# ryanelandt/PressureFieldContact.jl

Hardware: AMD Instinct MI355X
Metric: tet-tri clip+integrate ops/s (higher is better)
Workload: dtype f64

## Files before the change

### pressurefieldcontact.jl_amd/csrc/pfc_hip.hip

```cpp
#include "pfc_kernels.h"

#include <atomic>
#include <condition_variable>
#include <functional>
#include <mutex>
#include <thread>
#include <cmath>
#include <cstdlib>
#include <limits>
#include <cstdarg>
#include <cstdio>
#include <cstring>
#include <string>
#include <vector>

#include "../../include/pfc.h"
#include "pfc_sort.h"

namespace pfc {

__global__ void k_prep_tri(int n, const double *__restrict__ pt, const int *__restrict__ tri, TriRec *__restrict__ out) {
    int k = blockIdx.x * blockDim.x + threadIdx.x;
    if (k >= n) return;
    V3 a = ld3(pt + 3 * tri[3 * k]), b = ld3(pt + 3 * tri[3 * k + 1]), c = ld3(pt + 3 * tri[3 * k + 2]);
// ... 329 lines not shown
    hipStream_t last_stream = nullptr;
    long long stats[8] = {0, 0, 0, 0, 0, 0, 0, 0};
    DevBuf<double> dual_in, dual_acc, dual_res, dual_out, dual_poly;
    DevBuf<int2> dual_pkey;
    DevBuf<int> dual_sel, dual_flag;
    DevBuf<double> scat_d;
    DevBuf<int> scat_i;
    DevBuf<double> sdual_d, sdual_w;
    DevBuf<int> sdual_i;
    DevBuf<char> sdual_tmp;
    DevBuf<int> surv;
    DevBuf<int> rgn;
    DevBuf<int> poly_item, pcnt, poly_cand;
    DevBuf<double> poly;
    long long last_undecided = 0;
    long long last_active = 0;
    struct ShapeHint { int n = 0; bool sparse = false; } hints[4];
    void note_shape(int n, bool sparse) {
        int k = 0;
        while (k < 3 && hints[k].n != n) ++k;
        for (; k > 0; --k) hints[k] = hints[k - 1];
        hints[0].n = n; hints[0].sparse = sparse;
    }
    bool shape_is_sparse(int n) const {
        for (const ShapeHint &e : hints) if (e.n == n) return e.sparse;
        return false;
    }
    long long last_tslots = 0;
    Event ev[EV_COUNT];
    bool ev_valid = false;
    pfc_context *twin = nullptr;
    bool is_twin = false;
    DevBuf<int> fout;
    PinBuf<int> h_fout;
    int *fout_dev = nullptr;
    const int *fout_host = nullptr;
    int opt_fused = 1;
    int opt_fixed_order = 0;
    DevBuf<int> det;
    DevBuf<unsigned long long> sort_keys[2];
    DevBuf<int> canon_off, canon_fill, canon_item;
    int sort_tmp_items = 0;
    bool fixed_whole_list = false;
    DevBuf<char> sort_tmp;
    size_t sort_tmp_for = 0;
    int sort_tmp_bits = 0;
    int max_elem1 = 1, max_elem2 = 1;
    DevBuf<double> fx_rec, vfx_rec;
    DevBuf<int> vfx_head;
    DevBuf<int> fx_head;
    long long surv_sorted_serial = -1;
    size_t sort_cover = 0;
    size_t sort_cover_used = 0;
    int opt_clip_queue = 1;
    int fused_skip = 0;
    int fused_seq = 0;
    int fu_nw = 1;
    int last_fu_nw = 0, last_team = 0;
    int n_cu = 0;
    int opt_team = 48;
    DevBuf<unsigned long long> team;
    DevBuf<int> emit_ctr;
    PinBuf<int> h_emit;
    PinBuf<unsigned> h_more;
    bool fu_emit = false;
    int dual_fused_skip = 0;
    const double *fu_dpose = nullptr, *fu_dtwist = nullptr;
    double *fu_dwrench = nullptr, *fu_dsdot = nullptr;
    int fu_ndir = 0;
    bool pending_fused = false, last_fused = false;
    int opt_split_min = 1025;
    int opt_clip_min = 384;
    int opt_poison = 0;
    int split_n0 = 0;
    bool in_split = false;
    int last_parts = 1;
    Event ev_fork, ev_join, ev_join0;
    int twin_queue_fallback = 0;
    DevBuf<long long> surf_cnt, surf_off, surf_out;
    DevBuf<double> surf_part;
    DevBuf<int> surf_seg, surf_canon_off, surf_canon_fill, surf_canon_item;
    DevBuf<double> ljac_seed;
    DevBuf<double> ljac_out;
    DevBuf<double> ljac_io;
    DevBuf<int> ljac_ids;
    DevBuf<unsigned long long> surf_keys[2];
    DevBuf<char> surf_tmp;
    PinBuf<long long> h_surf;
    bool pending_surface = false;
    bool surf_whole_list = false;
    bool surf_cap_short = false;
    int surf_n_ctr = 0;
    long long surf_cap_poly = 0, surf_cap_trac = 0;
    DevBuf<long long> surf_hl;
    DevBuf<int> surf_hi;
    DevBuf<double> surf_hd, surf_in;
    size_t surf_hcap_poly = 0, surf_hcap_trac = 0;
    DevBuf<double> sfric_mom, sfric_sum, sfric_res;
    DevBuf<double> sfric_hd;
};

namespace {

int fail(pfc_context *h, int code, const char *fmt, ...) {
    char buf[512];
    va_list ap;
// ... 278 lines not shown
    } else if (np_mode == 0) {
        if (h->any_tet_tet) hipLaunchKernelGGL((k_narrow<true, 0>), dim3(np_grid), dim3(kNpBlock), 0, st, np);
        else hipLaunchKernelGGL((k_narrow<false, 0>), dim3(np_grid), dim3(kNpBlock), 0, st, np);
    } else {
        if (h->opt_clip_queue && !h->any_tet_tet) {
            hipLaunchKernelGGL(k_clip_queue, dim3(np_grid), dim3(kNpBlock), 0, st, np);
        } else if (h->in_split || (n_items >= 640 && n_items < 1024)) {
            if (h->any_tet_tet) hipLaunchKernelGGL((k_narrow<true, 3>), dim3(np_grid), dim3(kNpBlock), 0, st, np);
            else hipLaunchKernelGGL((k_narrow<false, 3>), dim3(np_grid), dim3(kNpBlock), 0, st, np);
        } else {
            if (h->any_tet_tet) hipLaunchKernelGGL((k_narrow<true, 2>), dim3(np_grid), dim3(kNpBlock), 0, st, np);
            else hipLaunchKernelGGL((k_narrow<false, 2>), dim3(np_grid), dim3(kNpBlock), 0, st, np);
        }
        IntegArgs ig;
        ig.items = h->items.p; ig.n_items = n_items; ig.ccount = ccount; ig.ccap = (int)h->ccap; ig.chunk_switch = kNpChunkSwitch;
        ig.pcnt = h->pcnt.p; ig.poly_item = h->poly_item.p; ig.poly = h->poly.p; ig.pcap = np.pcap;
        ig.poly_cand = np.poly_cand; ig.surv = np.surv; ig.scount = np.scount; ig.acc = h->acc.p; ig.rec = h->rec.p;
        ig.rgn = h->rgn.p; ig.rr_cap = np.rr_cap; ig.icnt = h->icnt.p; ig.status = h->status.p;
        ig.det = h->opt_fixed_order ? h->det.p : nullptr;
        if (h->opt_fixed_order) hipLaunchKernelGGL(k_integ_fixed, dim3(grid_for(h->ccap, 64, kNpMaxBlocks)), dim3(64), 0, st, ig);
        else hipLaunchKernelGGL(k_integ, dim3(grid_for(h->ccap, 64, kNpMaxBlocks)), dim3(64), 0, st, ig);
    }
    if (prof) HIP_TRY(h, hipEventRecord(h->ev[EV_NP], st));

    BrArgs br;
    br.items = h->items.p; br.n_items = n_items; br.acc = h->acc.p; br.res = h->res.p; br.icnt = h->icnt.p;
    br.trac = trac_view(h); br.tcount = tcount; br.tcap = (int)h->tcap; br.wrench = d_wrench; br.sdot = d_sdot;
    br.counts = d_counts;
    br.ctr = h->ctr.p; br.n_ctr = levels + 12; br.status = h->status.p; br.tail = h->tail_dev ? h->tail_dev : h->tail.p;
    br.rgn = h->rgn.p; br.i_pcount = (levels + 9) & ~1;
    if (h->opt_fixed_order && np_mode == 2) {
        FixedArgs fx;
        fx.rec = h->rec.p; fx.det = h->det.p; fx.n_items = n_items; fx.n_slots = (int)(h->rcap / kRgn) * kRgn; fx.items = h->items.p;
        fx.acc = h->acc.p; fx.status = h->status.p;
        hipLaunchKernelGGL(k_shift_fixed, dim3(n_items), dim3(64), 0, st, fx);
    }
    if (h->any_bristle) {
        ShiftArgs sh;
        sh.rec = h->rec.p; sh.rgn = h->rgn.p; sh.rr_cap = (int)(h->rcap / kRgn); sh.acc = h->acc.p;
        if (!(h->opt_fixed_order && np_mode == 2)) hipLaunchKernelGGL(k_shift, dim3(grid_for(h->rcap, 64, 2048)), dim3(64), 0, st, sh);
        hipLaunchKernelGGL(k_eig, dim3(n_items), dim3(64), 0, st, br);
        FricArgs fr;
        fr.items = h->items.p; fr.poly_item = h->poly_item.p; fr.poly = h->poly.p; fr.ccount = ccount; fr.ccap = (int)h->ccap;
        fr.chunk_switch = kNpChunkSwitch; fr.pcnt = h->pcnt.p;
        fr.pcap = np.pcap; fr.res = h->res.p; fr.acc = h->acc.p;
        fr.n_items = n_items; fr.status = h->status.p;
        fr.sink = FixedSink{nullptr, nullptr, nullptr, 0, 0, 0, 0, 0, nullptr};
        if (h->opt_fixed_order && np_mode == 2) {
            const size_t n_pos = h->ccap / 64 + 1, cap = fixed_fric_cap(h->ccap, n_items);
            HIP_TRY(h, hipMemsetAsync(h->vfx_head.p, 0xFF, sizeof(int) * (size_t)n_items, st));
            HIP_TRY(h, hipMemsetAsync(h->vfx_head.p + n_items, 0, sizeof(int) * 2, st));
            fr.sink = FixedSink{h->vfx_rec.p, h->vfx_head.p + n_items, h->vfx_head.p, 0, 2, (int)n_pos, (int)(2 * n_pos), (int)cap, h->status.p};
        }
        if (fr.sink.rec) {
            hipLaunchKernelGGL(k_fric_fixed, dim3(grid_for(h->ccap, 64, 256 * 32)), dim3(64), 0, st, fr);
            hipLaunchKernelGGL(k_fixed_reduce, dim3(n_items), dim3(64), 0, st, fr.sink, n_items, h->acc.p, kAccStride, kAccFric, 6);
        } else hipLaunchKernelGGL(k_fric, dim3(grid_for(h->ccap, 64, 256 * 32)), dim3(64), 0, st, fr);
    }
    if (prof) HIP_TRY(h, hipEventRecord(h->ev[EV_BR], st));
    hipLaunchKernelGGL(k_final, dim3(grid_for(n_items, 128, 1 << 20)), dim3(128), 0, st, br);
    if (prof) HIP_TRY(h, hipEventRecord(h->ev[EV_FIN], st));
    HIP_TRY(h, hipGetLastError());
    return PFC_OK;
}

int enqueue_eval(pfc_context *h, int n_items, const int *d_ins_ids, const double *d_pose, const double *d_twist,
                 const double *d_s, double *d_wrench, double *d_sdot, int *d_counts, hipStream_t st) {
    new_value_pass(h);
    h->pending_more = false; h->last_dual_reused = false;
    HIP_TRY(h, ensure_work(h, n_items));
    const int levels = eff_levels(h);
    const bool prof = h->opt_profile != 0;
    if (prof && !h->ev[0])
        for (int k = 0; k < EV_COUNT; ++k) HIP_TRY(h, hipEventCreate(h->ev[k].put()));
    const int L = bfs_levels_for(h, n_items, levels);
    bool use_graph = h->opt_graph && !prof;
#ifdef PFC_STAMPS
    use_graph = false;
#endif
    if (use_graph) {
        pfc_context::GraphKey key = {};
        key.n_items = n_items; key.levels = levels; key.L = L; key.debug = (h->opt_debug ? 1 : 0) | (h->in_split ? 2 : 0) | (bp_block_for(h, n_items) << 4);
        if (h->opt_fixed_order) {
            size_t cover = h->sort_cover ? h->sort_cover : h->ccap;
            int lg = 0;
            while (((size_t)1 << lg) < cover && lg < 40) ++lg;
            key.debug |= ((lg + 1) << 16) | (h->fixed_whole_list ? 1 << 24 : 0);
        }
        key.bristle = (h->any_bristle ? 1 : 0) | (h->any_tet_tet ? 2 : 0);
        key.surv = h->want_surv ? 1 : 0;
        key.p[0] = d_ins_ids; key.p[1] = d_pose; key.p[2] = d_twist; key.p[3] = d_s; key.p[4] = d_wrench;
        key.p[5] = d_sdot; key.p[6] = d_counts; key.p[7] = h->tail_dev; key.p[8] = h->bp_dev; key.stream = (void *)st; key.epoch = h->epoch;
        const int gi = key.surv;
        if (!h->ghave[gi] || std::memcmp(&key, &h->gkey[gi], sizeof key) != 0) {
            h->gexec[gi].reset();
            h->ghave[gi] = false;
            hipGraph_t graph = nullptr;
            HIP_TRY(h, hipStreamBeginCapture(st, hipStreamCaptureModeThreadLocal));
            int rc = record_eval(h, n_items, d_ins_ids, d_pose, d_twist, d_s, d_wrench, d_sdot, d_counts, st, false);
            hipError_t e = hipStreamEndCapture(st, &graph);
            if (rc != PFC_OK) { if (graph) (void)hipGraphDestroy(graph); return rc; }
            if (e != hipSuccess) return fail(h, PFC_ERR_HIP, "hipStreamEndCapture failed: %s", hipGetErrorString(e));
            e = hipGraphInstantiate(h->gexec[gi].put(), graph, nullptr, nullptr, 0);
            (void)hipGraphDestroy(graph);
            if (e != hipSuccess) return fail(h, PFC_ERR_HIP, "hipGraphInstantiate failed: %s", hipGetErrorString(e));
            h->gkey[gi] = key; h->ghave[gi] = true;
        }
        HIP_TRY(h, hipGraphLaunch(h->gexec[gi], st));
    } else {
        int rc = record_eval(h, n_items, d_ins_ids, d_pose, d_twist, d_s, d_wrench, d_sdot, d_counts, st, prof);
// ... 672 lines not shown
        HIP_TRY(h, copy_sync(h, h->d_insfull, full.data(), sizeof(InsFull) * full.size(), hipMemcpyHostToDevice));
    }
    h->finalized = true;
    return PFC_OK;
}

static int check_eval_args(pfc_context *h, int n_items, const void *ins_ids, const void *pose, const void *twist,
                           const void *s, const void *wrench, const void *sdot) {
    if (!h->finalized) return fail(h, PFC_ERR_STATE, "pfc_eval before pfc_finalize");
    if (n_items < 0) return fail(h, PFC_ERR_BAD_ARG, "negative n_items");
    if (n_items == 0) return PFC_OK;
    if (h->ins.empty()) return fail(h, PFC_ERR_STATE, "no contact instructions");
    if (!pose || !twist || !wrench || !sdot) return fail(h, PFC_ERR_BAD_ARG, "null buffer");
    if (!ins_ids && n_items > (int)h->ins.size())
        return fail(h, PFC_ERR_BAD_ARG, "n_items exceeds the number of instructions and no ins_ids given");
    if (h->any_bristle && !s) return fail(h, PFC_ERR_BAD_ARG, "bristle instructions need the state buffer s");
    return PFC_OK;
}

int pfc_eval_device(pfc_handle h, int n_items, const int *d_ins_ids, const double *d_pose, const double *d_twist,
                    const double *d_s, double *d_wrench, double *d_sdot, int *d_counts, void *stream) {
    if (!h) return PFC_ERR_BAD_ARG;
    if (h->multi)
        return multi_eval_device(h, n_items, 0, d_ins_ids, d_pose, nullptr, d_twist, d_s, nullptr, nullptr, nullptr, d_wrench, d_sdot,
                                 nullptr, nullptr, d_counts, stream);
    { const int rc = check_eval_args(h, n_items, d_ins_ids, d_pose, d_twist, d_s, d_wrench, d_sdot); if (rc != PFC_OK) return rc; }
    if (n_items == 0) { h->pending = false; h->last_n_items = 0; return PFC_OK; }
    HIP_TRY(h, hipSetDevice(h->device));
    hipStream_t st = stream ? (hipStream_t)stream : h->stream;
    h->split_n0 = 0;
    h->pending_fused = false;
    end_kept_pass(h);
    h->pending_more = false;
    int team = fused_team(h, n_items);
    if (team > 1 && !team_acquire(h)) team = fused_ok(h, n_items) ? 1 : 0;
    if (team) {
        h->fu_nw = team;
        const int rc_t = enqueue_fused(h, n_items, d_ins_ids, d_pose, d_twist, d_s, d_wrench, d_sdot, d_counts, st);
        h->fu_nw = 1;
        if (rc_t != PFC_OK) team_release(h);
        return rc_t;
    }
    if (h->fused_skip > 0 && n_items <= kFusedMaxItems) --h->fused_skip;
    const bool split = h->opt_split_min > 0 && n_items >= h->opt_split_min && d_ins_ids && !h->opt_debug && !h->opt_fixed_order &&
                       !h->want_surv && !h->is_twin && !pile_mode(h, n_items);
    if (!split) return enqueue_eval(h, n_items, d_ins_ids, d_pose, d_twist, d_s, d_wrench, d_sdot, d_counts, st);
    int rc = make_twin(h);
    if (rc != PFC_OK) return rc;
    pfc_context *t = h->twin;
    t->opt_profile = h->opt_profile; t->opt_max_levels = h->opt_max_levels; t->opt_bfs_levels = h->opt_bfs_levels;
    t->opt_poison = h->opt_poison;
    if (t->opt_clip_min != h->opt_clip_min) { t->opt_clip_min = h->opt_clip_min; t->ghave[0] = t->ghave[1] = false; }
    if (t->opt_clip_queue != h->opt_clip_queue) { t->opt_clip_queue = h->opt_clip_queue; t->ghave[0] = t->ghave[1] = false; }
    t->opt_graph = h->opt_graph;
    if (t->opt_no_filter != h->opt_no_filter) { t->opt_no_filter = h->opt_no_filter; t->ghave[0] = t->ghave[1] = false; }
    const int n0 = n_items / 2, n1 = n_items - n0;
    hipStream_t s0 = h->stream;
    HIP_TRY(h, hipEventRecord(h->ev_fork, st));
    if (s0 != st) HIP_TRY(h, hipStreamWaitEvent(s0, h->ev_fork, 0));
    HIP_TRY(h, hipStreamWaitEvent(t->stream, h->ev_fork, 0));
    h->in_split = true; t->in_split = true;
    rc = enqueue_eval(h, n0, d_ins_ids, d_pose, d_twist, d_s, d_wrench, d_sdot, d_counts, s0);
    h->in_split = false;
    if (rc != PFC_OK) return rc;
    rc = enqueue_eval(t, n1, d_ins_ids + n0, d_pose + 24 * (size_t)n0, d_twist + 6 * (size_t)n0,
                      d_s ? d_s + 6 * (size_t)n0 : nullptr, d_wrench + 6 * (size_t)n0, d_sdot + 6 * (size_t)n0,
                      d_counts ? d_counts + 4 * (size_t)n0 : nullptr, t->stream);
    if (rc != PFC_OK) { h->err = t->err; return rc; }
    HIP_TRY(h, hipEventRecord(h->ev_join, t->stream));
    HIP_TRY(h, hipStreamWaitEvent(st, h->ev_join, 0));
    if (s0 != st) {
        HIP_TRY(h, hipEventRecord(h->ev_join0, s0));
        HIP_TRY(h, hipStreamWaitEvent(st, h->ev_join0, 0));
    }
    h->split_n0 = n0;
    return PFC_OK;
}

namespace {

struct SurfFricOut {
    const double *s;
    double *fric, *fric_summary, *stiff;
};

int surface_enqueue(pfc_context *h, int n_items, const int *d_ins_ids, const double *d_pose, const double *d_twist, long long cap_poly,
                    long long cap_trac, long long *d_poly_off, int *d_poly_idx, double *d_poly_xyz, long long *d_poly_trac,
                    double *d_trac, double *d_summary, int *d_counts, long long *d_totals, hipStream_t st, const SurfFricOut *fo = nullptr) {
    new_value_pass(h);
    h->pending_more = false;
    h->pin_in_pt = {}; h->pin_din_pt = {};
    h->pending = false; h->pending_dual = false; h->pending_dual_hyb = false; h->split_n0 = 0;
    if (h->pending_fused) { h->pending_fused = false; team_release(h); }
    int ba, bb;
    const int bits = pfc_sort_key_bits(n_items, h->max_elem1, h->max_elem2, &ba, &bb);
    if (bits > 64)
        return fail(h, PFC_ERR_BAD_ARG, "pfc_contact_surface: (item, element, element) needs %d key bits for %d items, more than 64", bits, n_items);
    HIP_TRY(h, ensure_work(h, n_items));
    const size_t c = h->ccap;
    HIP_TRY(h, h->surf_cnt.ensure(2 * (c + 1)));
    HIP_TRY(h, h->surf_off.ensure(2 * (c + 1)));
    HIP_TRY(h, h->surf_part.ensure(c * kSurfSums));
    HIP_TRY(h, h->surf_seg.ensure((size_t)n_items + 1));
    HIP_TRY(h, h->surf_canon_off.ensure((size_t)n_items + 1));
    HIP_TRY(h, h->surf_canon_fill.ensure((size_t)n_items));
    HIP_TRY(h, h->surf_canon_item.ensure(c));
// ... 1172 lines not shown
        copy_out_dual(po + n * 12, nk, d_wrench, d_sdot);
        h->dual_counts_cache.assign(pc, pc + n * 4);
        h->pin_din_pt = {n_items, ins_ids != nullptr, h->value_serial, in_d};
        return PFC_OK;
    }
    h->want_surv = true;
    int rc = pfc_eval(h, n_items, ins_ids, pose, twist, s, wrench, sdot, counts);
    h->want_surv = false;
    if (rc != PFC_OK) return rc;
    HIP_TRY(h, ensure_graphed(h, h->dual_in, nk * 36));
    HIP_TRY(h, ensure_graphed(h, h->dual_acc, nk * kDaStride));
    HIP_TRY(h, ensure_graphed(h, h->dual_res, nk * kDrStride));
    HIP_TRY(h, ensure_graphed(h, h->dual_out, nk * 12));
    double *dp = h->dual_in.p, *dt = dp + nk * 24, *dsd = dt + nk * 6;
    const size_t in_bytes = sizeof(double) * nk * 36, out_bytes = sizeof(double) * nk * 12;
    HIP_TRY(h, h->pin_in.ensure(in_bytes));
    HIP_TRY(h, h->pin_out.ensure(out_bytes));
    pack_seeds((double *)h->pin_in.p, nk, d_pose, d_twist, d_s, true);
    HIP_TRY(h, hipMemcpyAsync(dp, h->pin_in.p, in_bytes, hipMemcpyHostToDevice, st));
    rc = launch_dual(h, n_items, n_dir, h->tail.p, dp, dt, dsd, h->dual_out.p, h->dual_out.p + nk * 6, (size_t)h->stats[2], st, nullptr);
    if (rc != PFC_OK) return rc;
    h->dual_hint = h->stats[2];
    HIP_TRY(h, hipMemcpyAsync(h->pin_out.p, h->dual_out.p, out_bytes, hipMemcpyDeviceToHost, st));
    HIP_TRY(h, hipStreamSynchronize(st));
    copy_out_dual((const double *)h->pin_out.p, nk, d_wrench, d_sdot);
    return PFC_OK;
}

int pfc_set_option(pfc_handle h, const char *name, long long value) {
    if (!h || !name) return PFC_ERR_BAD_ARG;
    if (h->multi) {
        if (!std::strcmp(name, "multi_min")) { h->multi->opt_min_items = value < 1 ? 1 : (int)value; h->multi->part_n = 0; return PFC_OK; }
        h->multi->dev_kept = false;
        for (pfc_context *c : h->multi->shard) {
            const int rc = on_shard(h, c, [&](pfc_context *c1) { return pfc_set_option(c1, name, value); });
            if (rc != PFC_OK) return rc;
        }
        return PFC_OK;
    }
    end_kept_pass(h);
    if (!std::strcmp(name, "debug")) h->opt_debug = value != 0;
    else if (!std::strcmp(name, "profile")) h->opt_profile = value != 0;
    else if (!std::strcmp(name, "max_levels")) {
        if (value < 0 || value > (1 << 20) || (h->finalized && value > h->max_levels))
            return fail(h, PFC_ERR_BAD_ARG, "max_levels must be 0 (automatic) or 1..%d (depth of the finalized trees + 1)", h->max_levels);
        h->opt_max_levels = (int)value; h->ghave[0] = h->ghave[1] = false; h->dghave = false;
    }
    else if (!std::strcmp(name, "bfs_levels")) h->opt_bfs_levels = (int)value;
    else if (!std::strcmp(name, "graph")) h->opt_graph = value != 0;
    else if (!std::strcmp(name, "split_min")) h->opt_split_min = (int)value;
    else if (!std::strcmp(name, "dual_reuse")) h->opt_dual_reuse = (int)value;
    else if (!std::strcmp(name, "clip_min")) { h->opt_clip_min = (int)value; h->ghave[0] = h->ghave[1] = false; h->dghave = false; }
    else if (!std::strcmp(name, "clip_queue")) { h->opt_clip_queue = (int)value; h->ghave[0] = h->ghave[1] = false; h->dghave = false; }
    else if (!std::strcmp(name, "poison")) h->opt_poison = value != 0;
    else if (!std::strcmp(name, "fused")) { h->opt_fused = value != 0; h->fused_skip = 0; }
    else if (!std::strcmp(name, "team")) h->opt_team = value < 0 ? 0 : (value > kTeamMaxWg ? kTeamMaxWg : (int)value);
    else if (!std::strcmp(name, "team_fault")) h->opt_team_fault = (int)value;
    else if (!std::strcmp(name, "fused_f32")) h->opt_fused_f32 = value != 0;
    else if (!std::strcmp(name, "dual_fold")) { h->opt_dual_fold = value != 0; h->dghave = false; }
    else if (!std::strcmp(name, "fixed_order")) {
        const int on = value != 0;
        if (on != h->opt_fixed_order) {
            h->opt_fixed_order = on; h->fused_skip = 0;
            h->ghave[0] = h->ghave[1] = false; h->dghave = false;
            h->rec.release();
        }
    }
    else if (!std::strcmp(name, "no_filter")) { h->opt_no_filter = (int)value; h->ghave[0] = h->ghave[1] = false; h->dghave = false; }
    else return fail(h, PFC_ERR_BAD_ARG, "unknown option %s", name);
    return PFC_OK;
}

int pfc_get_stats(pfc_handle h, long long *out8) {
    if (!h || !out8) return PFC_ERR_BAD_ARG;
    if (h->multi) { for (int k = 0; k < 8; ++k) out8[k] = h->multi->stats[k]; return PFC_OK; }
    for (int k = 0; k < 8; ++k) out8[k] = h->stats[k];
    return PFC_OK;
}

int pfc_get_stage_ms(pfc_handle h, float *out6) {
    if (!h || !out6) return PFC_ERR_BAD_ARG;
    if (h->multi)
        return on_first_shard(h, [&](pfc_context *c) { return pfc_get_stage_ms(c, out6); });
    if (!h->ev_valid) return fail(h, PFC_ERR_STATE, "profile option was off for the last evaluation");
    HIP_TRY(h, hipSetDevice(h->device));
    HIP_TRY(h, hipEventSynchronize(h->ev[EV_FIN]));
    for (int k = 0; k < 5; ++k) HIP_TRY(h, hipEventElapsedTime(&out6[k], h->ev[k], h->ev[k + 1]));
    HIP_TRY(h, hipEventElapsedTime(&out6[5], h->ev[EV_START], h->ev[EV_FIN]));
    if (h->last_parts == 2 && h->twin && h->twin->ev_valid) {
        pfc_context *t = h->twin;
        float b[6];
        HIP_TRY(h, hipEventSynchronize(t->ev[EV_FIN]));
        for (int k = 0; k < 5; ++k) HIP_TRY(h, hipEventElapsedTime(&b[k], t->ev[k], t->ev[k + 1]));
        HIP_TRY(h, hipEventElapsedTime(&b[5], t->ev[EV_START], t->ev[EV_FIN]));
        for (int k = 0; k < 5; ++k) out6[k] = 0.5f * (out6[k] + b[k]);
        if (b[5] > out6[5]) out6[5] = b[5];
    }
    return PFC_OK;
}

int pfc_last_parts(pfc_handle h) { return h ? (h->multi ? pfc_last_parts(h->multi->shard[0]) : (h->last_fused ? 0 : h->last_parts)) : 0; }
int pfc_last_team(pfc_handle h) { return h ? (h->multi ? pfc_last_team(h->multi->shard[0]) : (h->last_fused ? h->last_fu_nw : 0)) : 0; }
int pfc_last_dual_reused(pfc_handle h) {
    if (!h) return 0;
    if (h->multi) {
        for (int k = 0; k < h->multi->n_used; ++k)
// ... 330 lines not shown
```

### pressurefieldcontact.jl_amd/csrc/pfc_kernels.h

```cpp
#pragma once
#include <hip/hip_runtime.h>

namespace pfc {

constexpr int kInternal = -9999;
constexpr int kWave = 64;

enum : unsigned {
    kStNonFinite = 1u,
    kStFrontierOvf = 2u,
    kStCandOvf = 4u,
    kStTracOvf = 8u,
    kStBadIns = 16u,
    kStAbort = 32u,
    kStRecOvf = 64u,
    kStPolyOvf = 128u,
    kStHole = 256u,
    kStFixedSpan = 2048u,
    kStFixedCover = 8192u,
    kStFixedBig = 16384u,
    kStFixedList = 4096u,
};

struct alignas(16) NodeRec {
// ... 275 lines not shown
    else if (d2 >= d3) { q0 = R[6] - R[2]; q1 = R[3] + R[1]; q2 = d2; q3 = R[7] + R[5]; }
    else { q0 = R[1] - R[3]; q1 = R[6] + R[2]; q2 = R[7] + R[5]; q3 = d3; }
    const double qn = __builtin_sqrt(((q0 * q0 + q1 * q1) + q2 * q2) + q3 * q3);
    qf[0] = (float)(q0 / qn); qf[1] = (float)(q1 / qn); qf[2] = (float)(q2 / qn); qf[3] = (float)(q3 / qn);
    const double w = qf[0], x = qf[1], y = qf[2], z = qf[3];
    const double Rq[9] = {1 - 2 * (y * y + z * z), 2 * (x * y + z * w), 2 * (x * z - y * w),
                          2 * (x * y - z * w), 1 - 2 * (x * x + z * z), 2 * (y * z + x * w),
                          2 * (x * z + y * w), 2 * (y * z - x * w), 1 - 2 * (x * x + y * y)};
    double worst = 0.0;
#pragma unroll
    for (int j = 0; j < 9; ++j) worst = fmax(worst, __builtin_fabs(Rq[j] - R[j]));
    const double n2 = ((w * w + x * x) + y * y) + z * z;
    const double u = 5.9604644775390625e-8;
    return (worst <= 4.0 * u) && (__builtin_fabs(n2 - 1.0) <= 2.25 * u);
}

struct PointParams {
    V3 w, vl;
    double chi, Ebar, er0, er1, er2, er3;
    int nq;
};
template <class F>
__device__ __forceinline__ int fan_triangle_points(const PointParams &c, const V3 &v1, const V3 &v2, const V3 &cen, const V3 &nh,
                                                   F &&body) {
    const double area = triangle_area(v1, v2, cen, nh);
    if (!(0.0 < area)) return 0;
    int n_pt = 0;
    for (int q = 0; q < c.nq; ++q) {
        double q0, q1, q2, qw;
        if (c.nq == 1) {
            q0 = q1 = q2 = 0.33333333333333331483; qw = 1.0;
        } else {
            const double qa = 0.16666666666666674068, qb = 0.66666666666666651864;
            q0 = (q == 1) ? qb : qa; q1 = (q == 0) ? qb : qa; q2 = (q == 2) ? qb : qa;
            qw = 0.33333333333333331483;
        }
        const V3 r = mk3((v1.x * q0 + v2.x * q1) + cen.x * q2, (v1.y * q0 + v2.y * q1) + cen.y * q2,
                         (v1.z * q0 + v2.z * q1) + cen.z * q2);
        double eq = __builtin_fma(c.er0, r.x, c.er3);
        eq = __builtin_fma(c.er1, r.y, eq);
        eq = __builtin_fma(c.er2, r.z, eq);
        const V3 rdot = c.vl + cross(c.w, r);
        const double ee = -dot(mk3(c.er0, c.er1, c.er2), rdot);
        const double damp = fmax(0.0, 1.0 + c.chi * ee);
        const double p = eq * c.Ebar * damp;
        const double dA = qw * area;
        if (!(0.0 < p)) continue;
        ++n_pt;
        body(r, rdot, p, dA);
    }
    return n_pt;
}

__device__ __forceinline__ int sat15_f32_core(const float *ea, const float *eb, const float *t, const float *R, float E) {
    float aR[9];
#pragma unroll
    for (int k = 0; k < 9; ++k) aR[k] = __builtin_fabsf(R[k]);
    float dmax;
#define R_(i, j) R[(i) + 3 * (j)]
#define AR_(i, j) aR[(i) + 3 * (j)]
#define AXIS_(tl, rsum) dmax = __builtin_fmaxf(dmax, (tl) - (rsum))
    {
        const float rb = __builtin_fmaf(AR_(0, 2), eb[2], __builtin_fmaf(AR_(0, 1), eb[1], AR_(0, 0) * eb[0]));
        dmax = __builtin_fabsf(t[0]) - (ea[0] + rb);
    }
#pragma unroll
    for (int i = 1; i < 3; ++i) {
        const float rb = __builtin_fmaf(AR_(i, 2), eb[2], __builtin_fmaf(AR_(i, 1), eb[1], AR_(i, 0) * eb[0]));
        AXIS_(__builtin_fabsf(t[i]), ea[i] + rb);
    }
#pragma unroll
    for (int j = 0; j < 3; ++j) {
        const float tl = __builtin_fabsf(__builtin_fmaf(R_(2, j), t[2], __builtin_fmaf(R_(1, j), t[1], R_(0, j) * t[0])));
        const float ra = __builtin_fmaf(AR_(2, j), ea[2], __builtin_fmaf(AR_(1, j), ea[1], AR_(0, j) * ea[0]));
        AXIS_(tl, ra + eb[j]);
    }
    constexpr int i100[3] = {1, 0, 0}, i221[3] = {2, 2, 1};
#pragma unroll
    for (int j = 0; j < 3; ++j) {
        const float tl = __builtin_fabsf(__builtin_fmaf(t[2], R_(1, j), -(t[1] * R_(2, j))));
        const float ra = __builtin_fmaf(ea[1], AR_(2, j), ea[2] * AR_(1, j));
        const float rb = __builtin_fmaf(eb[i100[j]], AR_(0, i221[j]), eb[i221[j]] * AR_(0, i100[j]));
        AXIS_(tl, ra + rb);
    }
#pragma unroll
    for (int j = 0; j < 3; ++j) {
        const float tl = __builtin_fabsf(__builtin_fmaf(t[0], R_(2, j), -(t[2] * R_(0, j))));
        const float ra = __builtin_fmaf(ea[0], AR_(2, j), ea[2] * AR_(0, j));
        const float rb = __builtin_fmaf(eb[i100[j]], AR_(1, i221[j]), eb[i221[j]] * AR_(1, i100[j]));
        AXIS_(tl, ra + rb);
    }
#pragma unroll
    for (int j = 0; j < 3; ++j) {
        const float tl = __builtin_fabsf(__builtin_fmaf(t[1], R_(0, j), -(t[0] * R_(1, j))));
        const float ra = __builtin_fmaf(ea[0], AR_(1, j), ea[1] * AR_(0, j));
        const float rb = __builtin_fmaf(eb[i100[j]], AR_(2, i221[j]), eb[i221[j]] * AR_(2, i100[j]));
        AXIS_(tl, ra + rb);
    }
#undef AXIS_
#undef R_
#undef AR_
    return (dmax > E) ? 0 : ((dmax < -E) ? 1 : 2);
}

template <bool CONJ_A>
__device__ __forceinline__ void quat_mul(const float *a, const float *b, float *r) {
// ... 181 lines not shown
```

### pressurefieldcontact.jl_amd/csrc/pfc_np.h

```cpp
#pragma once

struct TracSoA {
    int *item;
    double *nx, *ny, *nz, *rx, *ry, *rz, *dA, *p;
};

struct NpArgs {
    const ItemRec *items;
    const WorkRec *cand;
    const int *ccount;
    int ccap;
    double *acc;
    double *rec;
    int *rgn;
    int rr_cap;
    int *pcnt;
    int chunk_switch;
    int *poly_cand;
    int *icnt;
    int n_items;
    int *clip_n;
    int *poly_item;
    double *poly;
    int pcap;
// ... 1118 lines not shown
                    M27_(0, W * nh.x * nh.x); M27_(1, W * nh.x * nh.y); M27_(2, W * nh.x * nh.z);
                    M27_(3, W * nh.y * nh.y); M27_(4, W * nh.y * nh.z); M27_(5, W * nh.z * nh.z);
                    const V3 an = cross(m1, nh);
                    M27_(6, an.x * nh.x); M27_(7, an.y * nh.x); M27_(8, an.z * nh.x);
                    M27_(9, an.x * nh.y); M27_(10, an.y * nh.y); M27_(11, an.z * nh.y);
                    M27_(12, an.x * nh.z); M27_(13, an.y * nh.z); M27_(14, an.z * nh.z);
                    const V3 q0c = mk3(q[0], q[1], q[2]), q1c = mk3(q[1], q[3], q[4]), q2c = mk3(q[2], q[4], q[5]);
                    const V3 m0 = cross(nh, q0c), m1c = cross(nh, q1c), m2c = cross(nh, q2c);
                    const V3 r0 = cross(nh, mk3(m0.x, m1c.x, m2c.x)), r1 = cross(nh, mk3(m0.y, m1c.y, m2c.y));
                    const V3 r2 = cross(nh, mk3(m0.z, m1c.z, m2c.z));
                    M27_(15, r0.x); M27_(16, r0.y); M27_(17, r0.z); M27_(18, r1.y); M27_(19, r1.z); M27_(20, r2.z);
#pragma unroll
                    for (int k = 0; k < 6; ++k) M27_(21 + k, q[k]);
#undef M27_
                }
            }
            if (has && (!contributed || lane_reg)) g.poly_item[idx] = 0;
            if (g.surv != nullptr) {
                const unsigned long long sm = __ballot(has);
                if (sm) {
                    int sbase = 0;
                    if (lane == 0) sbase = atomicAdd(g.scount, __popcll(sm));
                    sbase = __builtin_amdgcn_readfirstlane(sbase);
                    if (has) g.surv[sbase + __popcll(sm & ((1ull << lane) - 1ull))] = contributed ? g.poly_cand[idx] : -1;
                }
            }
        }
        flush();
    }
}
__global__ void __launch_bounds__(64, 2) k_integ(IntegArgs g) {
    __shared__ double m27[27 * 66];
    integ_body<false>(g, m27);
}
__global__ void __launch_bounds__(64, 2) k_integ_fixed(IntegArgs g) {
    __shared__ double m27[27 * 66];
    integ_body<true>(g, m27);
}

struct FricArgs {
    const ItemRec *items;
    const int *poly_item;
    const double *poly;
    const int *ccount;
    int ccap, chunk_switch;
    const int *pcnt;
    int pcap;
    int n_items;
    unsigned *status;
    const double *res;
    double *acc;
    FixedSink sink;
};
template <bool FX>
__device__ __forceinline__ void fric_body(const FricArgs &g) {
    const int lane = threadIdx.x;
    const size_t P = (size_t)g.pcap;
    int n_c = *g.ccount;
    if (n_c > g.ccap) n_c = g.ccap;
    const int C = np_chunk(n_c, g.chunk_switch);
    const int n_chunk = (n_c + C - 1) / C;
    for (int ch = blockIdx.x; ch < n_chunk; ch += gridDim.x) {
      int cnt = __builtin_amdgcn_readfirstlane(g.pcnt[ch]);
      if (cnt > C) cnt = C;
      for (int p0 = 0; p0 < cnt; p0 += 64) {
        const int idx = ch * C + p0 + lane;
        const bool active = p0 + lane < cnt;
        double sum[6];
#pragma unroll
        for (int k = 0; k < 6; ++k) sum[k] = 0.0;
        int item = 0;
        bool contributed = false;
        unsigned pk = active ? (unsigned)g.poly_item[idx] : 0u;
        if ((pk >> 28) > 8u || ((pk >> 28) >= 3u && (pk & 0x0FFFFFFFu) >= (unsigned)g.n_items)) {
            atomicOr(g.status, kStHole);
            pk = 0u;
        }
        if ((pk >> 28) >= 3u) {
            item = (int)(pk & 0x0FFFFFFFu);
            const int n = (int)(pk >> 28);
            const ItemRec *it = g.items + item;
            const double *o = g.poly + idx;
            const V3 nh = mk3(o[0], o[P], o[2 * P]);
            const V3 cen = mk3(o[3 * P], o[4 * P], o[5 * P]);
            const double er0 = o[6 * P], er1 = o[7 * P], er2 = o[8 * P], er3 = o[9 * P];
            const int nq = it->nq;
            const V3 w = ld3(it->w), vl = ld3(it->v);
            const double chi = it->chi, Ebar = it->Ebar, mu_s = it->mu_s, mu_d = it->mu_d;
            const double tau = it->tau, k_bar = it->k_bar;
            const double mu_slope = (mu_d - mu_s) / (3 * mu_s - 2 * mu_s);
            const double *res = g.res + (size_t)item * kResStride;
            const V3 cop = ld3(res + kResCop), Da = ld3(res + kResDelta), Dl = ld3(res + kResDelta + 3);
            const V3 ts_c0 = ((Dl - cross(Da, cop)) + vl * tau) * (-k_bar), ts_e = (Da + w * tau) * (-k_bar);
            V3 v2 = mk3(o[(10 + 3 * (n - 1)) * P], o[(11 + 3 * (n - 1)) * P], o[(12 + 3 * (n - 1)) * P]);
            V3 vn = mk3(o[10 * P], o[11 * P], o[12 * P]);
            PointParams pp;
            pp.w = w; pp.vl = vl; pp.chi = chi; pp.Ebar = Ebar; pp.er0 = er0; pp.er1 = er1; pp.er2 = er2; pp.er3 = er3; pp.nq = nq;
            for (int k = 0; k < n; ++k) {
                const V3 v1 = v2;
                v2 = vn;
                if (k + 1 < n) vn = mk3(o[(13 + 3 * k) * P], o[(14 + 3 * k) * P], o[(15 + 3 * k) * P]);
                if (fan_triangle_points(pp, v1, v2, cen, nh, [&](const V3 &r, const V3 &, double p, double dA) {
                    const double p_dA = p * dA;
                    const V3 x = r - cop;
                    V3 Ts = ts_c0 + cross_fma(ts_e, r);
                    Ts = axpy_fma(-dot_fma(Ts, nh), nh, Ts);
                    const double m2 = dot_fma(Ts, Ts);
                    V3 T;
                    if (m2 < mu_s * mu_s) {
                        T = Ts;
                    } else {
                        double ri = __builtin_amdgcn_rsq(m2);
                        const double hm = 0.5 * m2;
                        ri = ri * __builtin_fma(-hm * ri, ri, 1.5);
                        ri = ri * __builtin_fma(-hm * ri, ri, 1.5);
                        const double mg = m2 * ri;
                        const double y = mu_s + (mg - 2 * mu_s) * mu_slope;
                        const double mu = (y > mu_s) ? mu_s : ((y < mu_d) ? mu_d : y);
                        T = Ts * (mu * ri);
                    }
                    const V3 Tc = T * p_dA;
                    const V3 ta = cross_fma(x, Tc);
                    sum[0] += ta.x; sum[1] += ta.y; sum[2] += ta.z;
                    sum[3] += Tc.x; sum[4] += Tc.y; sum[5] += Tc.z;
                }))
                    contributed = true;
            }
        }
        accumulate_items<6, FX>(g.acc, item, FX ? (active && (pk >> 28) >= 3u) : active, contributed, sum, kAccFric, kAccStride, &g.sink, (ch * C + p0) >> 6);
      }
    }
}
__global__ void __launch_bounds__(64, 3) k_fric(FricArgs g) { fric_body<false>(g); }
__global__ void __launch_bounds__(64, 3) k_fric_fixed(FricArgs g) { fric_body<true>(g); }
```

Measured before the change: 3.986 billion.

## Compute friction quadrature points from per-corner linear fields in k_fric

Adds a templated path to the friction kernel that evaluates the pressure-field and trial-traction linear fields once per fan corner and the centroid. Quadrature-point values are then formed as weighted combinations of those corner values, so the generic per-point fan_triangle_points evaluation is no longer used. This is meant to cut redundant per-point arithmetic in the integration loop. It is enabled by default through a new vertex_fields option. It relies on the fields being exactly linear, which can change rounding, and it adds a second kernel instantiation.

```diff
diff --git a/pressurefieldcontact.jl_amd/csrc/pfc_hip.hip b/pressurefieldcontact.jl_amd/csrc/pfc_hip.hip
--- a/pressurefieldcontact.jl_amd/csrc/pfc_hip.hip
+++ b/pressurefieldcontact.jl_amd/csrc/pfc_hip.hip
@@ -405,6 +405,7 @@
     long long surv_sorted_serial = -1;
     size_t sort_cover = 0;
     size_t sort_cover_used = 0;
+    int opt_vertex_fields = 1;
     int opt_clip_queue = 1;
     int fused_skip = 0;
     int fused_seq = 0;
@@ -789,10 +790,13 @@
             HIP_TRY(h, hipMemsetAsync(h->vfx_head.p + n_items, 0, sizeof(int) * 2, st));
             fr.sink = FixedSink{h->vfx_rec.p, h->vfx_head.p + n_items, h->vfx_head.p, 0, 2, (int)n_pos, (int)(2 * n_pos), (int)cap, h->status.p};
         }
+        const bool vertex_fields = h->opt_vertex_fields && !h->opt_debug;
         if (fr.sink.rec) {
-            hipLaunchKernelGGL(k_fric_fixed, dim3(grid_for(h->ccap, 64, 256 * 32)), dim3(64), 0, st, fr);
+            if (vertex_fields) hipLaunchKernelGGL(k_fric_fixed<true>, dim3(grid_for(h->ccap, 64, 256 * 32)), dim3(64), 0, st, fr);
+            else hipLaunchKernelGGL(k_fric_fixed<false>, dim3(grid_for(h->ccap, 64, 256 * 32)), dim3(64), 0, st, fr);
             hipLaunchKernelGGL(k_fixed_reduce, dim3(n_items), dim3(64), 0, st, fr.sink, n_items, h->acc.p, kAccStride, kAccFric, 6);
-        } else hipLaunchKernelGGL(k_fric, dim3(grid_for(h->ccap, 64, 256 * 32)), dim3(64), 0, st, fr);
+        } else if (vertex_fields) hipLaunchKernelGGL(k_fric<true>, dim3(grid_for(h->ccap, 64, 256 * 32)), dim3(64), 0, st, fr);
+        else hipLaunchKernelGGL(k_fric<false>, dim3(grid_for(h->ccap, 64, 256 * 32)), dim3(64), 0, st, fr);
     }
     if (prof) HIP_TRY(h, hipEventRecord(h->ev[EV_BR], st));
     hipLaunchKernelGGL(k_final, dim3(grid_for(n_items, 128, 1 << 20)), dim3(128), 0, st, br);
@@ -1571,6 +1575,7 @@
     t->opt_poison = h->opt_poison;
     if (t->opt_clip_min != h->opt_clip_min) { t->opt_clip_min = h->opt_clip_min; t->ghave[0] = t->ghave[1] = false; }
     if (t->opt_clip_queue != h->opt_clip_queue) { t->opt_clip_queue = h->opt_clip_queue; t->ghave[0] = t->ghave[1] = false; }
+    if (t->opt_vertex_fields != h->opt_vertex_fields) { t->opt_vertex_fields = h->opt_vertex_fields; t->ghave[0] = t->ghave[1] = false; }
     t->opt_graph = h->opt_graph;
     if (t->opt_no_filter != h->opt_no_filter) { t->opt_no_filter = h->opt_no_filter; t->ghave[0] = t->ghave[1] = false; }
     const int n0 = n_items / 2, n1 = n_items - n0;
@@ -2849,6 +2854,10 @@
     else if (!std::strcmp(name, "dual_reuse")) h->opt_dual_reuse = (int)value;
     else if (!std::strcmp(name, "clip_min")) { h->opt_clip_min = (int)value; h->ghave[0] = h->ghave[1] = false; h->dghave = false; }
     else if (!std::strcmp(name, "clip_queue")) { h->opt_clip_queue = (int)value; h->ghave[0] = h->ghave[1] = false; h->dghave = false; }
+    else if (!std::strcmp(name, "vertex_fields")) {
+        if (value != 0 && value != 1) return fail(h, PFC_ERR_BAD_ARG, "vertex_fields must be 0 (per-point k_fric) or 1 (per-corner fields)");
+        h->opt_vertex_fields = (int)value; h->ghave[0] = h->ghave[1] = false; h->dghave = false;
+    }
     else if (!std::strcmp(name, "poison")) h->opt_poison = value != 0;
     else if (!std::strcmp(name, "fused")) { h->opt_fused = value != 0; h->fused_skip = 0; }
     else if (!std::strcmp(name, "team")) h->opt_team = value < 0 ? 0 : (value > kTeamMaxWg ? kTeamMaxWg : (int)value);
diff --git a/pressurefieldcontact.jl_amd/csrc/pfc_kernels.h b/pressurefieldcontact.jl_amd/csrc/pfc_kernels.h
--- a/pressurefieldcontact.jl_amd/csrc/pfc_kernels.h
+++ b/pressurefieldcontact.jl_amd/csrc/pfc_kernels.h
@@ -351,6 +351,45 @@
     return n_pt;
 }
 
+struct FanFields {
+    double er0, er1, er2, er3;
+    double d0;
+    V3 dg;
+    double qa, qd, qw;
+    int nq;
+};
+__device__ __forceinline__ FanFields fan_fields(const PointParams &c) {
+    FanFields f;
+    f.er0 = c.er0; f.er1 = c.er1; f.er2 = c.er2; f.er3 = c.er3;
+    const V3 e = mk3(c.er0, c.er1, c.er2);
+    f.d0 = __builtin_fma(-c.chi, dot(e, c.vl), 1.0);
+    f.dg = cross(e, c.w) * (-c.chi);
+    f.nq = c.nq;
+    if (c.nq == 1) { f.qa = 0.33333333333333331483; f.qd = 0.0; f.qw = 1.0; }
+    else { f.qa = 0.16666666666666674068; f.qd = 0.66666666666666651864 - 0.16666666666666674068; f.qw = 0.33333333333333331483; }
+    return f;
+}
+__device__ __forceinline__ double fan_field_a(const FanFields &f, const V3 &c) {
+    return __builtin_fma(f.er2, c.z, __builtin_fma(f.er1, c.y, __builtin_fma(f.er0, c.x, f.er3)));
+}
+__device__ __forceinline__ double fan_field_d(const FanFields &f, const V3 &c) {
+    return __builtin_fma(f.dg.z, c.z, __builtin_fma(f.dg.y, c.y, __builtin_fma(f.dg.x, c.x, f.d0)));
+}
+__device__ __forceinline__ double fan_linear_a(const FanFields &f, const V3 &r) {
+    return __builtin_fma(f.er2, r.z, __builtin_fma(f.er1, r.y, f.er0 * r.x));
+}
+__device__ __forceinline__ double fan_linear_d(const FanFields &f, const V3 &r) {
+    return __builtin_fma(f.dg.z, r.z, __builtin_fma(f.dg.y, r.y, f.dg.x * r.x));
+}
+__device__ __forceinline__ double fan_sum(const FanFields &f, double f1, double f2, double fc) { return __builtin_fma(f.qa, f1 + f2, fc); }
+__device__ __forceinline__ V3 fan_sum(const FanFields &f, const V3 &f1, const V3 &f2, const V3 &fc) {
+    return mk3(fan_sum(f, f1.x, f2.x, fc.x), fan_sum(f, f1.y, f2.y, fc.y), fan_sum(f, f1.z, f2.z, fc.z));
+}
+__device__ __forceinline__ double fan_at(const FanFields &f, double S, double corner) { return __builtin_fma(f.qd, corner, S); }
+__device__ __forceinline__ V3 fan_at(const FanFields &f, const V3 &S, const V3 &corner) {
+    return mk3(fan_at(f, S.x, corner.x), fan_at(f, S.y, corner.y), fan_at(f, S.z, corner.z));
+}
+
 __device__ __forceinline__ int sat15_f32_core(const float *ea, const float *eb, const float *t, const float *R, float E) {
     float aR[9];
 #pragma unroll
diff --git a/pressurefieldcontact.jl_amd/csrc/pfc_np.h b/pressurefieldcontact.jl_amd/csrc/pfc_np.h
--- a/pressurefieldcontact.jl_amd/csrc/pfc_np.h
+++ b/pressurefieldcontact.jl_amd/csrc/pfc_np.h
@@ -1194,7 +1194,7 @@
     double *acc;
     FixedSink sink;
 };
-template <bool FX>
+template <bool FX, bool VF>
 __device__ __forceinline__ void fric_body(const FricArgs &g) {
     const int lane = threadIdx.x;
     const size_t P = (size_t)g.pcap;
@@ -1238,6 +1238,58 @@
             V3 vn = mk3(o[10 * P], o[11 * P], o[12 * P]);
             PointParams pp;
             pp.w = w; pp.vl = vl; pp.chi = chi; pp.Ebar = Ebar; pp.er0 = er0; pp.er1 = er1; pp.er2 = er2; pp.er3 = er3; pp.nq = nq;
+            if constexpr (VF) {
+                const FanFields ff = fan_fields(pp);
+                const double mu_s2 = mu_s * mu_s;
+                const double a_c = fan_field_a(ff, cen), d_c = fan_field_d(ff, cen);
+                const V3 Ts_c0 = ts_c0 + cross_fma(ts_e, cen);
+                const V3 ts_c = axpy_fma(-dot_fma(Ts_c0, nh), nh, Ts_c0);
+                const V3 x_c = cen - cop;
+                struct Corner { V3 c, r; double a, d; V3 ts; };
+                auto corner = [&](const V3 &c) {
+                    Corner f;
+                    f.c = c; f.r = c - cen;
+                    f.a = fan_linear_a(ff, f.r); f.d = fan_linear_d(ff, f.r);
+                    const V3 Ts = cross_fma(ts_e, f.r);
+                    f.ts = axpy_fma(-dot_fma(Ts, nh), nh, Ts);
+                    return f;
+                };
+                Corner f2 = corner(v2);
+                for (int k = 0; k < n; ++k) {
+                    const Corner f1 = f2;
+                    f2 = corner(vn);
+                    if (k + 1 < n) vn = mk3(o[(13 + 3 * k) * P], o[(14 + 3 * k) * P], o[(15 + 3 * k) * P]);
+                    const double area = triangle_area(f1.c, f2.c, cen, nh);
+                    if (!(0.0 < area)) continue;
+                    const double dA = ff.qw * area;
+                    const double Sa = fan_sum(ff, f1.a, f2.a, a_c), Sd = fan_sum(ff, f1.d, f2.d, d_c);
+                    const V3 Sts = fan_sum(ff, f1.ts, f2.ts, ts_c), Sx = fan_sum(ff, f1.r, f2.r, x_c);
+                    auto point = [&](double eq, double d, const V3 &Ts, const V3 &x) {
+                        const double p = eq * Ebar * fmax(0.0, d);
+                        if (!(0.0 < p)) return;
+                        contributed = true;
+                        const double m2 = dot_fma(Ts, Ts);
+                        double sc = p * dA;
+                        if (!(m2 < mu_s2)) {
+                            double ri = __builtin_amdgcn_rsq(m2);
+                            const double hm = 0.5 * m2;
+                            ri = ri * __builtin_fma(-hm * ri, ri, 1.5);
+                            ri = ri * __builtin_fma(-hm * ri, ri, 1.5);
+                            const double mg = m2 * ri;
+                            const double y = mu_s + (mg - 2 * mu_s) * mu_slope;
+                            const double mu = (y > mu_s) ? mu_s : ((y < mu_d) ? mu_d : y);
+                            sc *= mu * ri;
+                        }
+                        const V3 xt = cross_fma(x, Ts);
+                        sum[0] = __builtin_fma(sc, xt.x, sum[0]); sum[1] = __builtin_fma(sc, xt.y, sum[1]);
+                        sum[2] = __builtin_fma(sc, xt.z, sum[2]); sum[3] = __builtin_fma(sc, Ts.x, sum[3]);
+                        sum[4] = __builtin_fma(sc, Ts.y, sum[4]); sum[5] = __builtin_fma(sc, Ts.z, sum[5]);
+                    };
+                    auto at = [&](const Corner &q) { point(fan_at(ff, Sa, q.a), fan_at(ff, Sd, q.d), fan_at(ff, Sts, q.ts), fan_at(ff, Sx, q.r)); };
+                    at(f2);
+                    if (ff.nq != 1) { at(f1); point(Sa, Sd, Sts, Sx); }
+                }
+            } else {
             for (int k = 0; k < n; ++k) {
                 const V3 v1 = v2;
                 v2 = vn;
@@ -1268,10 +1320,11 @@
                 }))
                     contributed = true;
             }
+            }
         }
         accumulate_items<6, FX>(g.acc, item, FX ? (active && (pk >> 28) >= 3u) : active, contributed, sum, kAccFric, kAccStride, &g.sink, (ch * C + p0) >> 6);
       }
     }
 }
-__global__ void __launch_bounds__(64, 3) k_fric(FricArgs g) { fric_body<false>(g); }
-__global__ void __launch_bounds__(64, 3) k_fric_fixed(FricArgs g) { fric_body<true>(g); }
+template <bool VF> __global__ void __launch_bounds__(64, 3) k_fric(FricArgs g) { fric_body<false, VF>(g); }
+template <bool VF> __global__ void __launch_bounds__(64, 3) k_fric_fixed(FricArgs g) { fric_body<true, VF>(g); }
```

Result: faster. 4.114 billion (median of 6 runs) (+3.2%).
